# srihari-humbarwadi/retinanet-tensorflow2.x

Hardware: AMD Instinct MI355X
Metric: images/sec train, ResNet50-640 RetinaNet data-parallel step (encode + fwd + loss + bwd + clip + all-reduce + SGD/EMA); inference images/s under `infer` (higher is better)
Workload: dtype bf16; 1 GPU; ResNet50-640x640 bf16 training, 32 images/GPU (BASELINE configs[2] shard: global batch 32), resnet_initial frozen, single GPU; global_batch=32, parallelism=dp1, rccl_ranks=1, comm=torch, syncbn_messages=0

## Files before the change

retinanet-tensorflow2.x_amd/csrc/rn_train.hip:

```cpp
#include "rn_common.h"

#define TR_THREADS 256

struct bf8 { float v[8]; };
__device__ __forceinline__ bf8 unpack8(uint4 u) {
  bf8 r;
  r.v[0] = rn_bf16_to_f32((uint16_t)(u.x & 0xffffu)); r.v[1] = rn_bf16_to_f32((uint16_t)(u.x >> 16));
  r.v[2] = rn_bf16_to_f32((uint16_t)(u.y & 0xffffu)); r.v[3] = rn_bf16_to_f32((uint16_t)(u.y >> 16));
  r.v[4] = rn_bf16_to_f32((uint16_t)(u.z & 0xffffu)); r.v[5] = rn_bf16_to_f32((uint16_t)(u.z >> 16));
  r.v[6] = rn_bf16_to_f32((uint16_t)(u.w & 0xffffu)); r.v[7] = rn_bf16_to_f32((uint16_t)(u.w >> 16));
  return r;
}
__device__ __forceinline__ uint4 pack8(const bf8& r) {
  uint4 u;
  u.x = rn_pack_bf16x2(r.v[0], r.v[1]); u.y = rn_pack_bf16x2(r.v[2], r.v[3]);
  u.z = rn_pack_bf16x2(r.v[4], r.v[5]); u.w = rn_pack_bf16x2(r.v[6], r.v[7]);
  return u;
}
__device__ __forceinline__ float act_mask(float z, int act) {
  if (act == RN_ACT_RELU) return z > 0.0f ? 1.0f : 0.0f;
  if (act == RN_ACT_RELU6) return (z > 0.0f && z < 6.0f) ? 1.0f : 0.0f;
  return 1.0f;
}
__device__ __forceinline__ float act_mask_u(float u, int act) {
  if (act == RN_ACT_RELU) return u > 0.0f ? 1.0f : 0.0f;
  if (act == RN_ACT_RELU6) {
    const float ub = rn_rb(u);
    return (ub > 0.0f && ub < 6.0f) ? 1.0f : 0.0f;
  }
  return 1.0f;
}
__device__ __forceinline__ float act_deriv(float z, float u, int act) {
  if (act == RN_ACT_SWISH) {
    const float sg = 1.0f / (1.0f + __expf(-u));
    return sg + u * sg * (1.0f - sg);
  }
  return act_mask(z, act);
}

enum { G_GENERIC = 0, G_NONE = 1, G_U_RELU = 2, G_U_RELU6 = 3, G_Z_RELU = 4, G_Z_RELU6 = 5, G_SWISH = 6, G_MASK = 7,
       G_SWISH_RES = 8 };
__device__ __forceinline__ float bn_swish_input(float u, float res) { return rn_rb(rn_rb(u) + res); }
template <int G>
__device__ __forceinline__ float grad_gate(float dz, float z, float u, int act, bool from_u) {
  if (G == G_NONE || G == G_MASK) return dz;
  if (G == G_U_RELU) return u > 0.0f ? dz : 0.0f;
  if (G == G_U_RELU6) {
    const float ub = rn_rb(u);
    return (ub > 0.0f && ub < 6.0f) ? dz : 0.0f;
  }
  if (G == G_Z_RELU) return z > 0.0f ? dz : 0.0f;
  if (G == G_Z_RELU6) return (z > 0.0f && z < 6.0f) ? dz : 0.0f;
  if (G == G_SWISH || G == G_SWISH_RES) {
    const float sg = __builtin_amdgcn_rcpf(1.0f + __expf(-u));
    return dz * (sg + u * sg * (1.0f - sg));
  }
  return act == RN_ACT_NONE ? dz : dz * (from_u ? act_mask_u(u, act) : act_deriv(z, u, act));
}
static int bn_gate_mode(const rn_bn_problem* p) {
  if (p->act == RN_ACT_NONE) return G_NONE;
  int with_res = 0;
  for (int i = 0; i < p->num_segments; ++i) with_res += p->seg[i].residual ? 1 : 0;
  if (with_res != 0 && with_res != p->num_segments) return G_GENERIC;
  if (p->act == RN_ACT_SWISH) return with_res ? G_SWISH_RES : G_SWISH;
  if (with_res == 0) return p->act == RN_ACT_RELU ? G_U_RELU : (p->act == RN_ACT_RELU6 ? G_U_RELU6 : G_GENERIC);
  int with_mask = 0;
  for (int i = 0; i < p->num_segments; ++i) with_mask += p->seg[i].act_mask ? 1 : 0;
  if (with_mask == p->num_segments && (p->act == RN_ACT_RELU || p->act == RN_ACT_RELU6)) return G_MASK;
  return p->act == RN_ACT_RELU ? G_Z_RELU : (p->act == RN_ACT_RELU6 ? G_Z_RELU6 : G_GENERIC);
}
#define BN_DISPATCH_GATE(mode_, CALL_)                  \
  switch (mode_) {                                      \
    case G_NONE: CALL_(G_NONE); break;                  \
    case G_U_RELU: CALL_(G_U_RELU); break;              \
    case G_U_RELU6: CALL_(G_U_RELU6); break;            \
    case G_Z_RELU: CALL_(G_Z_RELU); break;              \
    case G_Z_RELU6: CALL_(G_Z_RELU6); break;            \
    case G_SWISH: CALL_(G_SWISH); break;                \
    case G_MASK: CALL_(G_MASK); break;                  \
    case G_SWISH_RES: CALL_(G_SWISH_RES); break;        \
    default: CALL_(G_GENERIC); break;                   \
  }

static int tr_blocks(long long items, int cap = 8192) {
  long long b = rn_cdiv(items, TR_THREADS);
  if (b > cap) b = cap;
  if (b < 1) b = 1;
  return (int)b;
}

struct BnSegDev {
  const uint4* y; uint4* z; const uint4* residual; const uint4* dz; uint4* dy; uint4* dres;
  float* sums; float* fwd; float* bsums;
  const float* gamma; const float* beta; float* moving_mean; float* moving_var; float* dgamma; float* dbeta;
  long long P;
  int C, dres_accumulate, chunks, rows_per_chunk;
  int slab_groups, nslab;
  const float* sample_scale; long long rows_per_sample;
  unsigned char* mask;
  float* colsum;
};
struct BnArgs {
  int nseg, act, bessel, mode, fuse_finalize;
  int chunk_u;
  float eps, momentum, count_scale;
  float* ws;
  long long ws_off[RN_CONV_MAX_SEGMENTS];
  int ks[RN_CONV_MAX_SEGMENTS];
  long long cnt_off[RN_CONV_MAX_SEGMENTS], slot_off[RN_CONV_MAX_SEGMENTS], total_bytes;
  BnSegDev seg[RN_CONV_MAX_SEGMENTS];
};
#define BN_KS_MAX 32
#define BN_KS_CHUNKS 512

template <int G, int SGT = 0>
__global__ void __launch_bounds__(TR_THREADS) bn_colreduce_kernel(const BnArgs a) {
  const BnSegDev& s = a.seg[blockIdx.z];
  const int chunk = blockIdx.x;
  const int slab = blockIdx.y;
  if (chunk >= s.chunks || slab >= s.nslab) return;
  const int C8 = s.C >> 3;
  const int SG = SGT ? SGT : s.slab_groups, RL = TR_THREADS / SG;
  const int rl = threadIdx.x / SG, cg = threadIdx.x - rl * SG;
  const int c8 = slab * SG + cg;
  const bool live = c8 < C8 && rl < RL;
  const long long r0 = (long long)chunk * s.rows_per_chunk;
  long long r1 = r0 + s.rows_per_chunk;
  if (r1 > s.P) r1 = s.P;
  float s0[8], s1[8];
#pragma unroll
  for (int q = 0; q < 8; ++q) s0[q] = s1[q] = 0.0f;
  float mean[8], istd[8], scq[8], shq[8];
  if (G >= 0 && live) {
#pragma unroll
    for (int q = 0; q < 8; ++q) {
      mean[q] = s.fwd[0 * s.C + c8 * 8 + q];
      istd[q] = s.fwd[1 * s.C + c8 * 8 + q];
      scq[q] = s.fwd[2 * s.C + c8 * 8 + q];
      shq[q] = s.fwd[3 * s.C + c8 * 8 + q];
    }
  }
  if (live) {
    for (long long r = r0 + rl; r < r1; r += RL) {
      const long long o = r * C8 + c8;
      const bf8 y = unpack8(s.y[o]);
      if (G < 0) {
#pragma unroll
        for (int q = 0; q < 8; ++q) {
          s0[q] += y.v[q];
          s1[q] += y.v[q] * y.v[q];
        }
      } else {
        const bf8 dz = unpack8(s.dz[o]);
        const bool from_u = !s.residual && (a.act == RN_ACT_RELU || a.act == RN_ACT_RELU6);
        constexpr bool need_z = G == G_Z_RELU || G == G_Z_RELU6 || G == G_GENERIC;
        bf8 z;
        if (need_z && (G != G_GENERIC || (a.act != RN_ACT_NONE && a.act != RN_ACT_SWISH && !from_u))) z = unpack8(s.z[o]);
        unsigned bits = 0xffu;
        if (G == G_MASK) bits = s.mask[o];
        const bool swish_res = G == G_SWISH_RES || (G == G_GENERIC && a.act == RN_ACT_SWISH && s.residual != nullptr);
        bf8 res;
        if (swish_res) res = unpack8(s.residual[o]);
        float m = 1.0f;
        if (s.sample_scale) m = s.sample_scale[(int)r / (int)s.rows_per_sample];
#pragma unroll
        for (int q = 0; q < 8; ++q) {
          float u = y.v[q] * scq[q] + shq[q];
          if (swish_res) u = bn_swish_input(u, res.v[q]);
          float g = grad_gate<G < 0 ? 0 : G>(dz.v[q], z.v[q], u, a.act, from_u) * m;
          if (G == G_MASK) g = ((bits >> q) & 1u) ? g : 0.0f;
          s0[q] += g;
          s1[q] += g * ((y.v[q] - mean[q]) * istd[q]);
        }
      }
    }
  }
  __shared__ float red[SGT == 8 ? 2 * 32 * 65 : 2 * (TR_THREADS * 8 + TR_THREADS)];
  const int W = SG * 8 + 1;
  if (rl < RL) {
#pragma unroll
    for (int q = 0; q < 8; ++q) {
      red[rl * W + cg * 8 + q] = s0[q];
      red[RL * W + rl * W + cg * 8 + q] = s1[q];
    }
  }
  __syncthreads();
  for (int t = threadIdx.x; t < 2 * SG * 8; t += TR_THREADS) {
    const int which = t >= SG * 8 ? 1 : 0, c = t - which * SG * 8;
    float v = 0.0f;
    for (int r = 0; r < RL; ++r) v += red[which * RL * W + r * W + c];
    const int ch = slab * SG * 8 + c;
    if (ch < s.C) a.ws[a.ws_off[blockIdx.z] + ((long long)chunk * 2 + which) * s.C + ch] = v;
  }
}

static void bn_slab_plan(int C8, int chunks, int* slab_groups, int* nslab) {
  const int old_n = (C8 + 7) / 8;
  auto score = [&](int n) {
    const int g = (C8 + n - 1) / n;
    return (double)C8 * (TR_THREADS / g) / ((double)n * TR_THREADS);
  };
  *slab_groups = C8 < 8 ? C8 : 8;
  *nslab = old_n;
  if (C8 >= 8 && (double)C8 / (8.0 * old_n) >= 0.95) return;
  double best = 0.0;
  for (int n = 1; n <= old_n; ++n) {
    const int g = (C8 + n - 1) / n;
    if (g > 64 || (g < 8 && n > 1)) continue;
    if (score(n) > best) best = score(n);
  }
  for (int n = 1; n <= old_n; ++n) {
    const int g = (C8 + n - 1) / n;
    if (g > 64 || (g < 8 && n > 1) || score(n) < best - 0.01) continue;
    if ((long long)chunks * n >= 512 || C8 < 8) {
      *slab_groups = g;
      *nslab = n;
      return;
    }
  }
}

__device__ __forceinline__ void bn_finalize_channel(const BnArgs& a, const BnSegDev& s, int c, double sum, double sumsq) {
  const double n = (double)s.P * (double)a.count_scale;
  const double mean = sum / n;
  double var = sumsq / n - mean * mean;
  if (var < 0.0) var = 0.0;
  const float istd = (float)(1.0 / sqrt(var + (double)a.eps));
  const float sc = s.gamma[c] * istd;
  s.fwd[0 * s.C + c] = (float)mean;
  s.fwd[1 * s.C + c] = istd;
  s.fwd[2 * s.C + c] = sc;
  s.fwd[3 * s.C + c] = s.beta[c] - (float)mean * sc;
  if (s.moving_mean) {
    const double vm = a.bessel && n > 1.0 ? var * n / (n - 1.0) : var;
    s.moving_mean[c] = s.moving_mean[c] * a.momentum + (float)mean * (1.0f - a.momentum);
    s.moving_var[c] = s.moving_var[c] * a.momentum + (float)vm * (1.0f - a.momentum);
  }
}

template <int CH>
__global__ void __launch_bounds__(1024) bn_colreduce_final_kernel(const BnArgs a) {
  constexpr int LANES = 1024 / CH, PER = LANES / 16;
  const BnSegDev& s = a.seg[blockIdx.y];
  __shared__ double red[2][LANES][CH + 1];
  __shared__ double red2[2][16][CH + 1];
  const int cl = threadIdx.x & (CH - 1), lane = threadIdx.x / CH;
  const int c = blockIdx.x * CH + cl;
  double t0 = 0.0, t1 = 0.0;
  if (c < s.C) {
    const float* p = a.ws + a.ws_off[blockIdx.y];
#pragma unroll 8
    for (int k = lane; k < s.chunks; k += LANES) {
      t0 += (double)p[((long long)k * 2 + 0) * s.C + c];
      t1 += (double)p[((long long)k * 2 + 1) * s.C + c];
    }
  }
  red[0][lane][cl] = t0;
  red[1][lane][cl] = t1;
  __syncthreads();
  if (threadIdx.x < 2 * 16 * CH) {
    const int which = threadIdx.x / (16 * CH), rem = threadIdx.x - which * (16 * CH);
    const int grp = rem / CH, ch = rem - grp * CH;
    double t = 0.0;
#pragma unroll
    for (int j = 0; j < PER; ++j) t += red[which][grp * PER + j][ch];
    red2[which][grp][ch] = t;
  }
  __syncthreads();
  if (threadIdx.x < 2 * CH) {
    const int which = threadIdx.x / CH, ch = threadIdx.x - which * CH;
    const int cc = blockIdx.x * CH + ch;
    if (cc < s.C) {
      double t = 0.0;
#pragma unroll
      for (int j = 0; j < 16; ++j) t += red2[which][j][ch];
      float* out = a.mode == 0 ? s.sums : s.bsums;
      out[which * s.C + cc] = (float)t;
      if (a.mode == 1) {
        float* gp = which == 0 ? s.dbeta : s.dgamma;
        if (gp) gp[cc] = (float)t;
      }
      red2[which][0][ch] = (double)(float)t;
    }
  }
  if (a.fuse_finalize) {
    __syncthreads();
    if (threadIdx.x < CH && c < s.C) bn_finalize_channel(a, s, c, red2[0][0][cl], red2[1][0][cl]);
  }
}

typedef unsigned bn_u32x2_t __attribute__((ext_vector_type(2)));
__global__ void __launch_bounds__(1024) bn_colreduce_final_split_kernel(const BnArgs a) {
  const BnSegDev& s = a.seg[blockIdx.y];
  const int ks = a.ks[blockIdx.y], part = blockIdx.z;
  if (part >= ks || (int)blockIdx.x * 16 >= s.C) return;
  __shared__ double red[16][2][16];
  __shared__ unsigned s_old;
  const int col = threadIdx.x & 3, lane = threadIdx.x >> 2, wave = threadIdx.x >> 6;
  const int c = blockIdx.x * 16 + col * 4;
  double t[8];
#pragma unroll
  for (int q = 0; q < 8; ++q) t[q] = 0.0;
  if (c < s.C) {
    const float* p = a.ws + a.ws_off[blockIdx.y] + c;
    const int per = (s.chunks + ks - 1) / ks;
    const int k1 = (part + 1) * per < s.chunks ? (part + 1) * per : s.chunks;
#pragma unroll 2
    for (int k = part * per + lane; k < k1; k += 256) {
      const float4 v0 = *(const float4*)(p + ((long long)k * 2 + 0) * s.C);
      const float4 v1 = *(const float4*)(p + ((long long)k * 2 + 1) * s.C);
      t[0] += (double)v0.x; t[1] += (double)v0.y; t[2] += (double)v0.z; t[3] += (double)v0.w;
      t[4] += (double)v1.x; t[5] += (double)v1.y; t[6] += (double)v1.z; t[7] += (double)v1.w;
    }
  }
#pragma unroll
  for (int m = 4; m < 64; m <<= 1)
#pragma unroll
    for (int q = 0; q < 8; ++q) t[q] += __shfl_xor(t[q], m, 64);
  if ((threadIdx.x & 63) < 4) {
#pragma unroll
    for (int q = 0; q < 8; ++q) red[wave][q >> 2][col * 4 + (q & 3)] = t[q];
  }
  __syncthreads();
  const int which = (threadIdx.x >> 4) & 1, ch = threadIdx.x & 15;
  double r = 0.0;
  if (threadIdx.x < 32) {
#pragma unroll
    for (int j = 0; j < 16; ++j) r += red[j][which][ch];
  }
  if (ks > 1) {
    char* const slots = (char*)a.ws + a.slot_off[blockIdx.y] + (size_t)blockIdx.x * ks * 256;
    if (threadIdx.x < 64) {
      if (threadIdx.x < 32) {
        const __amdgpu_buffer_rsrc_t rs = __builtin_amdgcn_make_buffer_rsrc((void*)(slots + part * 256), 0, 256, 0x00020000);
        const unsigned long long bits = __builtin_bit_cast(unsigned long long, r);
        __builtin_amdgcn_raw_buffer_store_b64(bn_u32x2_t{(unsigned)bits, (unsigned)(bits >> 32)}, rs, threadIdx.x * 8, 0, 16);
      }
      asm volatile("s_waitcnt vmcnt(0)" ::: "memory");
      if (threadIdx.x == 0) {
        unsigned* const cnt = (unsigned*)((char*)a.ws + a.cnt_off[blockIdx.y]) + blockIdx.x;
        const unsigned old = __hip_atomic_fetch_add(cnt, 1u, __ATOMIC_RELAXED, __HIP_MEMORY_SCOPE_AGENT);
        if (old == (unsigned)(ks - 1)) __hip_atomic_store(cnt, 0u, __ATOMIC_RELAXED, __HIP_MEMORY_SCOPE_AGENT);
        s_old = old;
      }
    }
    __syncthreads();
    if (s_old != (unsigned)(ks - 1)) return;
    if (threadIdx.x < 32) {
      const __amdgpu_buffer_rsrc_t rs = __builtin_amdgcn_make_buffer_rsrc((void*)slots, 0, ks * 256, 0x00020000);
      bn_u32x2_t pv[BN_KS_MAX];
#pragma unroll
      for (int j = 0; j < BN_KS_MAX; ++j) pv[j] = __builtin_amdgcn_raw_buffer_load_b64(rs, j * 256 + threadIdx.x * 8, 0, 16);
      r = 0.0;
#pragma unroll
      for (int j = 0; j < BN_KS_MAX; ++j)
        r += __builtin_bit_cast(double, ((unsigned long long)pv[j].y << 32) | pv[j].x);
    }
  }
  if (threadIdx.x < 32) {
    const int cc = blockIdx.x * 16 + ch;
    if (cc < s.C) {
      float* out = a.mode == 0 ? s.sums : s.bsums;
      out[which * s.C + cc] = (float)r;
      if (a.mode == 1) {
        float* gp = which == 0 ? s.dbeta : s.dgamma;
        if (gp) gp[cc] = (float)r;
      }
    }
    red[0][which][ch] = (double)(float)r;
  }
  if (a.fuse_finalize) {
    __syncthreads();
    const int cc = blockIdx.x * 16 + threadIdx.x;
    if (threadIdx.x < 16 && cc < s.C) bn_finalize_channel(a, s, cc, red[0][0][threadIdx.x], red[0][1][threadIdx.x]);
  }
}

__global__ void bn_finalize_kernel(const BnArgs a) {
  const BnSegDev& s = a.seg[blockIdx.y];
  const int c = blockIdx.x * blockDim.x + threadIdx.x;
  if (c >= s.C) return;
  bn_finalize_channel(a, s, c, (double)s.sums[c], (double)s.sums[s.C + c]);
}

#define BN_ELEMENTWISE_RANGE() BN_ELEMENTWISE_RANGE_(false)
#define BN_ELEMENTWISE_RANGE_(keep_)                                                                  \
  long long first, last, step;                                                                        \
  if (a.chunk_u > 0) {                                                                                \
    const long long span = 256ll * a.chunk_u;                                                         \
    first = blockIdx.x * span + threadIdx.x;                                                          \
    last = (blockIdx.x + 1) * span < total ? (blockIdx.x + 1) * span : total;                         \
    step = 256;                                                                                       \
    if (first >= last) {                                                                              \
      if (!(keep_) || blockIdx.x * span >= total) return;    \
      first = last;                                                                                   \
    }                                                                                                 \
  } else {                                                                                            \
    const long long nthreads = (long long)gridDim.x * blockDim.x;                                     \
    step = nthreads / C8 * C8;                                                                        \
    first = blockIdx.x * (long long)blockDim.x + threadIdx.x;                                         \
    last = total;                                                                                     \
    if (first >= step) return;                                                                        \
  }

__global__ void __launch_bounds__(TR_THREADS) bn_apply_kernel(const BnArgs a) {
  const BnSegDev& s = a.seg[blockIdx.y];
  const int C8 = s.C >> 3;
  const long long total = s.P * C8;
  BN_ELEMENTWISE_RANGE();
  const int c8 = (int)(first % C8);
  float sc[8], sh[8];
#pragma unroll
  for (int q = 0; q < 8; ++q) {
    sc[q] = s.fwd[2 * s.C + c8 * 8 + q];
    sh[q] = s.fwd[3 * s.C + c8 * 8 + q];
  }
  for (long long i = first; i < last; i += step) {
    const bf8 y = unpack8(s.y[i]);
    bf8 o;
    bf8 res;
    if (s.residual) res = unpack8(s.residual[i]);
    const float m = s.sample_scale ? s.sample_scale[(int)(i / C8) / (int)s.rows_per_sample] : 1.0f;
    const bool swish = a.act == RN_ACT_SWISH;
#pragma unroll
    for (int q = 0; q < 8; ++q) o.v[q] = y.v[q] * sc[q] + sh[q];
    if (s.residual != nullptr || s.sample_scale != nullptr || swish) {
#pragma unroll
      for (int q = 0; q < 8; ++q) o.v[q] = rn_rb(o.v[q]);
    }
    if (s.sample_scale) {
#pragma unroll
      for (int q = 0; q < 8; ++q) o.v[q] = rn_rb(o.v[q] * m);
    }
    if (s.residual) {
#pragma unroll
      for (int q = 0; q < 8; ++q) o.v[q] += res.v[q];
      if (swish) {
#pragma unroll
        for (int q = 0; q < 8; ++q) o.v[q] = rn_rb(o.v[q]);
      }
    }
    rn_apply_act_n<8>(o.v, a.act);
    const uint4 zp = pack8(o);
    s.z[i] = zp;
    if (s.mask) {
      const bf8 zs = unpack8(zp);
      unsigned bits = 0u;
      if (a.act == RN_ACT_RELU) {
#pragma unroll
        for (int q = 0; q < 8; ++q) bits |= (zs.v[q] > 0.0f ? 1u : 0u) << q;
      } else if (a.act == RN_ACT_RELU6) {
#pragma unroll
        for (int q = 0; q < 8; ++q) bits |= ((zs.v[q] > 0.0f && zs.v[q] < 6.0f) ? 1u : 0u) << q;
      } else {
        bits = 0xffu;
      }
      s.mask[i] = (unsigned char)bits;
    }
  }
}

template <int G>
__global__ void __launch_bounds__(TR_THREADS) bn_bwd_apply_kernel(const BnArgs a) {
  const BnSegDev& s = a.seg[blockIdx.y];
  const int C8 = s.C >> 3;
  const long long total = s.P * C8;
  const float inv_n = (float)(1.0 / ((double)s.P * (double)a.count_scale));
  const bool colsum = s.colsum != nullptr;
  BN_ELEMENTWISE_RANGE_(colsum);
  const int c8 = a.chunk_u > 0 ? (int)(threadIdx.x % C8) : (int)(first % C8);
  float mean[8], istd[8], sc[8], shq[8], k1[8], k2[8];
#pragma unroll
  for (int q = 0; q < 8; ++q) {
    const int c = c8 * 8 + q;
    mean[q] = s.fwd[0 * s.C + c];
    istd[q] = s.fwd[1 * s.C + c];
    sc[q] = s.fwd[2 * s.C + c];
    shq[q] = s.fwd[3 * s.C + c];
    k1[q] = s.bsums[c] * inv_n;
    k2[q] = s.bsums[s.C + c] * inv_n;
  }
  float cs[8];
#pragma unroll
  for (int q = 0; q < 8; ++q) cs[q] = 0.0f;
  for (long long i = first; i < last; i += step) {
    const bf8 y = unpack8(s.y[i]);
    const bf8 dz = unpack8(s.dz[i]);
    const bool from_u = !s.residual && (a.act == RN_ACT_RELU || a.act == RN_ACT_RELU6);
    constexpr bool need_z = G == G_Z_RELU || G == G_Z_RELU6 || G == G_GENERIC;
    bf8 z;
    if (need_z && (G != G_GENERIC || (a.act != RN_ACT_NONE && a.act != RN_ACT_SWISH && !from_u))) z = unpack8(s.z[i]);
    const float m = s.sample_scale ? s.sample_scale[(int)(i / C8) / (int)s.rows_per_sample] : 1.0f;
    unsigned bits = 0xffu;
    if (G == G_MASK) bits = s.mask[i];
    const bool swish_res = G == G_SWISH_RES || (G == G_GENERIC && a.act == RN_ACT_SWISH && s.residual != nullptr);
    bf8 res;
    if (swish_res) res = unpack8(s.residual[i]);
    bf8 g, o;
#pragma unroll
    for (int q = 0; q < 8; ++q) {
      float u = y.v[q] * sc[q] + shq[q];
      if (swish_res) u = bn_swish_input(u, res.v[q]);
      g.v[q] = grad_gate<G>(dz.v[q], z.v[q], u, a.act, from_u);
      if (G == G_MASK) g.v[q] = ((bits >> q) & 1u) ? g.v[q] : 0.0f;
      const float xh = (y.v[q] - mean[q]) * istd[q];
      o.v[q] = sc[q] * (g.v[q] * m - k1[q] - xh * k2[q]);
    }
    const uint4 dyp = pack8(o);
    s.dy[i] = dyp;
    if (colsum) {
      const bf8 st = unpack8(dyp);
#pragma unroll
      for (int q = 0; q < 8; ++q) cs[q] += st.v[q];
    }
    if (s.dres) {
      if (s.dres_accumulate) {
        const bf8 old = unpack8(s.dres[i]);
#pragma unroll
        for (int q = 0; q < 8; ++q) g.v[q] += old.v[q];
      }
      s.dres[i] = pack8(g);
    }
  }
  if (colsum) {
    __shared__ float red[TR_THREADS][9];
#pragma unroll
    for (int q = 0; q < 8; ++q) red[threadIdx.x][q] = cs[q];
    __syncthreads();
    if ((int)threadIdx.x < C8) {
      float t[8];
#pragma unroll
      for (int q = 0; q < 8; ++q) t[q] = 0.0f;
      for (int j = threadIdx.x; j < TR_THREADS; j += C8)
#pragma unroll
        for (int q = 0; q < 8; ++q) t[q] += red[j][q];
      float* dst = s.colsum + ((long long)blockIdx.x * 2) * s.C + threadIdx.x * 8;
#pragma unroll
      for (int q = 0; q < 8; ++q) dst[q] = t[q];
    }
  }
}

static int bn_chunks_of(const rn_bn_segment& s, int mode, int* rows_per_chunk) {
  const long long want_chunks = 2048 / rn_cdiv(s.C, 64) < 256 ? 256 : 2048 / rn_cdiv(s.C, 64);
  long long rpc = rn_cdiv(rn_cdiv(s.P, want_chunks), 32) * 32;
  if (rpc < 32) rpc = 32;
  if (rows_per_chunk) *rows_per_chunk = (int)rpc;
  int chunks = (int)rn_cdiv(s.P, rpc);
  if (mode == 0 && s.ext_chunks > 0) chunks = s.ext_chunks;
  if (mode == 1 && s.ext_chunks_bwd > 0) chunks = s.ext_chunks_bwd;
  return chunks;
}

static int bn_fill(const rn_bn_problem* p, BnArgs& a, int need_ws, int mode = 1) {
  if (!p || p->num_segments < 1 || p->num_segments > RN_CONV_MAX_SEGMENTS) return -1;
  a.nseg = p->num_segments; a.act = p->act; a.bessel = p->bessel; a.mode = 0; a.fuse_finalize = 0; a.chunk_u = 0;
  a.eps = p->eps; a.momentum = p->momentum; a.count_scale = p->count_scale > 0 ? p->count_scale : 1.0f;
  long long off = 0;
  for (int i = 0; i < p->num_segments; ++i) {
    const rn_bn_segment& s = p->seg[i];
    if (s.P <= 0 || s.C <= 0 || (s.C % 8)) return -1;
    BnSegDev& d = a.seg[i];
    d.y = (const uint4*)s.y; d.z = (uint4*)s.z; d.residual = (const uint4*)s.residual;
    d.dz = (const uint4*)s.dz; d.dy = (uint4*)s.dy; d.dres = (uint4*)s.dres;
    d.sums = s.sums; d.fwd = s.fwd; d.bsums = s.bsums; d.gamma = s.gamma; d.beta = s.beta;
    d.moving_mean = s.moving_mean; d.moving_var = s.moving_var; d.dgamma = s.dgamma; d.dbeta = s.dbeta;
    d.P = s.P; d.C = s.C; d.dres_accumulate = s.dres_accumulate;
    d.sample_scale = s.sample_scale; d.rows_per_sample = s.rows_per_sample > 0 ? s.rows_per_sample : 1;
    d.mask = (unsigned char*)s.act_mask;
    d.colsum = s.dy_colsum_partial;
    if (s.sample_scale && p->act == RN_ACT_SWISH) return -1;
    d.chunks = bn_chunks_of(s, mode, &d.rows_per_chunk);
    bn_slab_plan(s.C / 8, d.chunks, &d.slab_groups, &d.nslab);
    a.ws_off[i] = off;
    off += (long long)d.chunks * 2 * s.C;
  }
  long long other = 0;
  for (int i = 0; i < p->num_segments; ++i) other += (long long)bn_chunks_of(p->seg[i], 1 - mode, nullptr) * 2 * p->seg[i].C;
  long long tail = ((off > other ? off : other) * 4 + 255) / 256 * 256;
  for (int i = 0; i < p->num_segments; ++i) {
    a.cnt_off[i] = tail;
    tail += rn_cdiv(p->seg[i].C, 16) * 4;
  }
  tail = (tail + 255) / 256 * 256;
  for (int i = 0; i < p->num_segments; ++i) {
    const int ch = a.seg[i].chunks;
    int ks = ch > BN_KS_CHUNKS ? (int)rn_cdiv(ch, 256) : 1;
    if (ks > BN_KS_MAX) ks = BN_KS_MAX;
    a.ks[i] = ks;
    a.slot_off[i] = tail;
    if (ks > 1) tail += rn_cdiv(p->seg[i].C, 16) * ks * 256;
  }
  a.total_bytes = tail;
  (void)need_ws;
  return 0;
}

extern "C" size_t rn_bn_workspace_bytes(const rn_bn_problem* p) {
  size_t need = 0;
  for (int mode = 0; mode < 2; ++mode) {
    BnArgs a;
    if (bn_fill(p, a, 1, mode)) return 0;
    if ((size_t)a.total_bytes > need) need = (size_t)a.total_bytes;
  }
  return need;
}

extern "C" int rn_bn_workspace_init(const rn_bn_problem* p, void* ws, size_t ws_bytes, void* stream) {
  BnArgs a;
  RN_CHECK_ARG(p && bn_fill(p, a, 1, 0) == 0, "rn_bn_workspace_init: bad problem (C %% 8 == 0, 1..10 segments)");
  const size_t need = rn_bn_workspace_bytes(p);
  if (!ws || ws_bytes < need) {
    rn_set_error("rn_bn_workspace_init: workspace too small (%zu < %zu)", ws_bytes, need);
    return RN_ENOMEM;
  }
  const long long begin = a.cnt_off[0];
  long long end = begin;
  for (int i = 0; i < p->num_segments; ++i) end = a.cnt_off[i] + rn_cdiv(p->seg[i].C, 16) * 4;
  RN_CHECK_HIP(hipMemsetAsync((char*)ws + begin, 0, (size_t)(end - begin), (hipStream_t)stream));
  return RN_OK;
}

extern "C" size_t rn_bn_partial_offset_bytes(const rn_bn_problem* p, int segment) {
  BnArgs a;
  if (bn_fill(p, a, 1, 0) || segment < 0 || segment >= a.nseg) return 0;
  return (size_t)a.ws_off[segment] * sizeof(float);
}

extern "C" size_t rn_bn_bwd_partial_offset_bytes(const rn_bn_problem* p, int segment) {
  BnArgs a;
  if (bn_fill(p, a, 1, 1) || segment < 0 || segment >= a.nseg) return 0;
  return (size_t)a.ws_off[segment] * sizeof(float);
}

static int bn_colreduce(const rn_bn_problem* p, int mode, void* ws, size_t ws_bytes, hipStream_t st,
                        const char* fn, int fuse_finalize = 0) {
  BnArgs a;
  RN_CHECK_ARG(bn_fill(p, a, 1, mode) == 0, "%s: bad problem (C %% 8 == 0, 1..10 segments)", fn);
  int n_ext = 0;
  for (int i = 0; i < p->num_segments; ++i)
    n_ext += ((mode == 0 && p->seg[i].ext_chunks > 0) || (mode == 1 && p->seg[i].ext_chunks_bwd > 0)) ? 1 : 0;
  RN_CHECK_ARG(n_ext == 0 || n_ext == p->num_segments, "%s: ext_chunks must be set on all segments or none", fn);
  if (mode == 1 && n_ext) {
    RN_CHECK_ARG(bn_gate_mode(p) == G_U_RELU, "%s: ext_chunks_bwd needs act = relu without residual inputs", fn);
    for (int i = 0; i < p->num_segments; ++i)
      RN_CHECK_ARG(!p->seg[i].sample_scale, "%s: ext_chunks_bwd with sample_scale", fn);
  }
  if (!ws || ws_bytes < rn_bn_workspace_bytes(p)) {
    rn_set_error("%s: workspace too small", fn);
    return RN_ENOMEM;
  }
  a.mode = mode;
  a.fuse_finalize = fuse_finalize;
  if (fuse_finalize)
    for (int i = 0; i < a.nseg; ++i)
      RN_CHECK_ARG(a.seg[i].fwd && a.seg[i].gamma && a.seg[i].beta, "%s: null tensor", fn);
  a.ws = (float*)ws;
  int max_chunks = 0, max_slabs = 0, max_c = 0;
  for (int i = 0; i < a.nseg; ++i) {
    const BnSegDev& s = a.seg[i];
    RN_CHECK_ARG(s.y && (mode == 0 ? s.sums != nullptr : (s.dz && s.bsums && s.fwd)), "%s: null tensor", fn);
    RN_CHECK_ARG(mode == 0 || a.act == RN_ACT_NONE || s.z || s.mask, "%s: z needed for the activation mask", fn);
    RN_CHECK_ARG(mode == 0 || bn_gate_mode(p) != G_GENERIC || a.act == RN_ACT_SWISH || !s.residual || s.z,
                 "%s: z needed for the activation mask", fn);
    if (s.chunks > max_chunks) max_chunks = s.chunks;
    if (s.nslab > max_slabs) max_slabs = s.nslab;
    if (s.C > max_c) max_c = s.C;
  }
  if (n_ext == 0) {
    const dim3 grid(max_chunks, max_slabs, a.nseg), block(TR_THREADS);
    bool all8 = true;
    for (int i = 0; i < a.nseg; ++i) all8 = all8 && a.seg[i].slab_groups == 8;
    if (mode == 0) {
      if (all8) hipLaunchKernelGGL((bn_colreduce_kernel<-1, 8>), grid, block, 0, st, a);
      else hipLaunchKernelGGL((bn_colreduce_kernel<-1, 0>), grid, block, 0, st, a);
    } else {
#define BN_CALL_(G_)                                                                       \
  if (all8) hipLaunchKernelGGL((bn_colreduce_kernel<G_, 8>), grid, block, 0, st, a);       \
  else hipLaunchKernelGGL((bn_colreduce_kernel<G_, 0>), grid, block, 0, st, a)
      BN_DISPATCH_GATE(bn_gate_mode(p), BN_CALL_)
#undef BN_CALL_
    }
    RN_CHECK_LAUNCH();
  }
  int max_ks = 1;
  for (int i = 0; i < a.nseg; ++i) max_ks = a.ks[i] > max_ks ? a.ks[i] : max_ks;
  if (max_ks > 1 && (((uintptr_t)a.ws) & 15) == 0)
    hipLaunchKernelGGL(bn_colreduce_final_split_kernel, dim3((max_c + 15) / 16, a.nseg, max_ks), dim3(1024), 0, st, a);
  else
    hipLaunchKernelGGL(bn_colreduce_final_kernel<16>, dim3((max_c + 15) / 16, a.nseg), dim3(1024), 0, st, a);
  RN_CHECK_LAUNCH();
  return RN_OK;
}

extern "C" int rn_bn_stats(const rn_bn_problem* p, void* ws, size_t ws_bytes, void* stream) {
  return bn_colreduce(p, 0, ws, ws_bytes, (hipStream_t)stream, "rn_bn_stats");
}
extern "C" int rn_bn_stats_finalize(const rn_bn_problem* p, void* ws, size_t ws_bytes, void* stream) {
  return bn_colreduce(p, 0, ws, ws_bytes, (hipStream_t)stream, "rn_bn_stats_finalize", 1);
}
extern "C" int rn_bn_bwd_reduce(const rn_bn_problem* p, void* ws, size_t ws_bytes, void* stream) {
  return bn_colreduce(p, 1, ws, ws_bytes, (hipStream_t)stream, "rn_bn_bwd_reduce");
}

extern "C" int rn_bn_finalize(const rn_bn_problem* p, void* stream) {
  BnArgs a;
  RN_CHECK_ARG(bn_fill(p, a, 0) == 0, "rn_bn_finalize: bad problem");
  int max_c = 0;
  for (int i = 0; i < a.nseg; ++i) {
    RN_CHECK_ARG(a.seg[i].sums && a.seg[i].fwd && a.seg[i].gamma && a.seg[i].beta, "rn_bn_finalize: null tensor");
    if (a.seg[i].C > max_c) max_c = a.seg[i].C;
  }
  hipLaunchKernelGGL(bn_finalize_kernel, dim3((max_c + 255) / 256, a.nseg), dim3(256), 0, (hipStream_t)stream, a);
  RN_CHECK_LAUNCH();
  return RN_OK;
}

#ifndef RN_BN_CHUNK_U
#define RN_BN_CHUNK_U 8
#endif
static int bn_elementwise_grid(BnArgs& a, long long max_units) {
  static_assert(TR_THREADS == 256, "BN_ELEMENTWISE_RANGE assumes 256 threads");
  bool chunk = RN_BN_CHUNK_U > 0;
  for (int i = 0; i < a.nseg; ++i) chunk = chunk && 256 % (a.seg[i].C >> 3) == 0;
  const long long blocks = rn_cdiv(max_units, 256ll * (RN_BN_CHUNK_U > 0 ? RN_BN_CHUNK_U : 1));
  if (chunk && blocks < (1ll << 31)) {
    a.chunk_u = RN_BN_CHUNK_U;
    return (int)blocks;
  }
  a.chunk_u = 0;
  return tr_blocks(max_units, 4096);
}

extern "C" int rn_bn_apply(const rn_bn_problem* p, void* stream) {
  BnArgs a;
  RN_CHECK_ARG(bn_fill(p, a, 0) == 0, "rn_bn_apply: bad problem");
  long long mx = 0;
  for (int i = 0; i < a.nseg; ++i) {
    RN_CHECK_ARG(a.seg[i].y && a.seg[i].z && a.seg[i].fwd, "rn_bn_apply: null tensor");
    const long long t = a.seg[i].P * (a.seg[i].C / 8);
    if (t > mx) mx = t;
  }
  hipLaunchKernelGGL(bn_apply_kernel, dim3(bn_elementwise_grid(a, mx), a.nseg), dim3(TR_THREADS), 0, (hipStream_t)stream, a);
  RN_CHECK_LAUNCH();
  return RN_OK;
}

extern "C" int rn_bn_bwd_colsum_chunks(const rn_bn_problem* p, int segment) {
  BnArgs a;
  if (bn_fill(p, a, 0) || segment < 0 || segment >= a.nseg) return 0;
  long long mx = 0;
  for (int i = 0; i < a.nseg; ++i) {
    const long long t = a.seg[i].P * (a.seg[i].C / 8);
    if (t > mx) mx = t;
  }
  bn_elementwise_grid(a, mx);
  if (a.chunk_u <= 0) return 0;
  return (int)rn_cdiv(a.seg[segment].P * (a.seg[segment].C / 8), 256ll * a.chunk_u);
}

extern "C" int rn_bn_bwd_apply(const rn_bn_problem* p, void* stream) {
  BnArgs a;
  RN_CHECK_ARG(bn_fill(p, a, 0) == 0, "rn_bn_bwd_apply: bad problem");
  long long mx = 0;
  for (int i = 0; i < a.nseg; ++i) {
    RN_CHECK_ARG(a.seg[i].y && a.seg[i].dz && a.seg[i].dy && a.seg[i].fwd && a.seg[i].bsums,
                 "rn_bn_bwd_apply: null tensor");
    RN_CHECK_ARG(a.act == RN_ACT_NONE || a.seg[i].z || a.seg[i].mask, "rn_bn_bwd_apply: z needed for the activation mask");
    RN_CHECK_ARG(bn_gate_mode(p) != G_GENERIC || a.act == RN_ACT_SWISH || !a.seg[i].residual || a.seg[i].z,
                 "rn_bn_bwd_apply: z needed for the activation mask");
    const long long t = a.seg[i].P * (a.seg[i].C / 8);
    if (t > mx) mx = t;
  }
  {
    const dim3 grid(bn_elementwise_grid(a, mx), a.nseg), block(TR_THREADS);
    for (int i = 0; i < a.nseg; ++i)
      RN_CHECK_ARG(!a.seg[i].colsum || a.chunk_u > 0,
                   "rn_bn_bwd_apply: dy_colsum_partial needs the chunked form (rn_bn_bwd_colsum_chunks() > 0)");
#define BN_CALL_(G_) hipLaunchKernelGGL(bn_bwd_apply_kernel<G_>, grid, block, 0, (hipStream_t)stream, a)
    BN_DISPATCH_GATE(bn_gate_mode(p), BN_CALL_)
#undef BN_CALL_
  }
  RN_CHECK_LAUNCH();
  return RN_OK;
}

__global__ void __launch_bounds__(TR_THREADS)
act_bwd_kernel(const uint4* __restrict__ dz, const uint4* __restrict__ z, uint4* __restrict__ dy, long long n8,
               int act) {
  for (long long i = blockIdx.x * (long long)blockDim.x + threadIdx.x; i < n8;
       i += (long long)gridDim.x * blockDim.x) {
    bf8 g = unpack8(dz[i]);
    const bf8 zz = unpack8(z[i]);
#pragma unroll
    for (int q = 0; q < 8; ++q) g.v[q] *= act_mask(zz.v[q], act);
    dy[i] = pack8(g);
  }
}

__global__ void __launch_bounds__(TR_THREADS)
cast_f32_bf16_kernel(const float4* __restrict__ x, uint2* __restrict__ y, long long n4) {
  for (long long i = blockIdx.x * (long long)blockDim.x + threadIdx.x; i < n4;
       i += (long long)gridDim.x * blockDim.x) {
    const float4 v = x[i];
    uint2 o;
    o.x = rn_pack_bf16x2(v.x, v.y);
    o.y = rn_pack_bf16x2(v.z, v.w);
    y[i] = o;
  }
}
__global__ void __launch_bounds__(TR_THREADS)
cast_pad_kernel(const float* __restrict__ x, uint2* __restrict__ y, long long P, int C, int Cpad) {
  const int q = Cpad / 4;
  const long long total = P * q;
  for (long long i = blockIdx.x * (long long)blockDim.x + threadIdx.x; i < total;
       i += (long long)gridDim.x * blockDim.x) {
    const long long r = i / q;
    const int c = (int)(i - r * q) * 4;
    float v[4];
#pragma unroll
    for (int u = 0; u < 4; ++u) v[u] = (c + u) < C ? x[r * C + c + u] : 0.0f;
    uint2 o;
    o.x = rn_pack_bf16x2(v[0], v[1]);
    o.y = rn_pack_bf16x2(v[2], v[3]);
    y[i] = o;
  }
}
extern "C" int rn_cast_pad_f32_to_bf16(const float* x, void* y, int64_t P, int C, int Cpad, void* stream) {
  RN_CHECK_ARG(x && y && P > 0 && C > 0 && Cpad >= C && Cpad % 4 == 0, "rn_cast_pad_f32_to_bf16: bad argument");
  hipLaunchKernelGGL(cast_pad_kernel, dim3(tr_blocks(P * (Cpad / 4))), dim3(TR_THREADS), 0, (hipStream_t)stream, x,
                     (uint2*)y, (long long)P, C, Cpad);
  RN_CHECK_LAUNCH();
  return RN_OK;
}
extern "C" int rn_cast_f32_to_bf16(const float* x, void* y, int64_t n, void* stream) {
  RN_CHECK_ARG(x && y && n > 0 && n % 4 == 0, "rn_cast_f32_to_bf16: bad argument (n %% 4 == 0)");
  hipLaunchKernelGGL(cast_f32_bf16_kernel, dim3(tr_blocks(n / 4)), dim3(TR_THREADS), 0, (hipStream_t)stream,
                     (const float4*)x, (uint2*)y, (long long)(n / 4));
  RN_CHECK_LAUNCH();
  return RN_OK;
}

__global__ void __launch_bounds__(TR_THREADS)
reduce_rows_kernel(const float* __restrict__ src, int rows, long long row_stride, int n, float add, float* __restrict__ dst) {
  const int c = blockIdx.x * blockDim.x + threadIdx.x;
  if (c >= n) return;
  float s = 0.0f;
  for (int r = 0; r < rows; ++r) s += src[r * row_stride + c];
  dst[c] = s + add;
}
extern "C" int rn_reduce_rows_f32(const float* src, int rows, int64_t row_stride, int n, float add, float* dst, void* stream) {
  RN_CHECK_ARG(src && dst && rows > 0 && n > 0 && row_stride >= 0, "rn_reduce_rows_f32: bad argument");
  hipLaunchKernelGGL(reduce_rows_kernel, dim3((n + TR_THREADS - 1) / TR_THREADS), dim3(TR_THREADS), 0, (hipStream_t)stream,
                     src, rows, (long long)row_stride, n, add, dst);
  RN_CHECK_LAUNCH();
  return RN_OK;
}

__global__ void __launch_bounds__(TR_THREADS)
upsample_zero_kernel(const uint4* __restrict__ x, uint4* __restrict__ y, int N, int H, int W, int C8, int Ho,
                     int Wo) {
  const long long total = (long long)N * Ho * Wo * C8;
  for (long long i = blockIdx.x * (long long)blockDim.x + threadIdx.x; i < total;
       i += (long long)gridDim.x * blockDim.x) {
    const RnIdx4 d_ = rn_decode4(i, C8, Wo, Ho, rn_decode_mode(total, C8));
    const int c = d_.c, ox = d_.x, oy = d_.y, n = d_.n;
    uint4 v = make_uint4(0u, 0u, 0u, 0u);
    if (!(ox & 1) && !(oy & 1) && (oy >> 1) < H && (ox >> 1) < W)
      v = x[(((long long)n * H + (oy >> 1)) * W + (ox >> 1)) * C8 + c];
    y[i] = v;
  }
}
extern "C" int rn_upsample_zero2x(const void* x, void* y, int N, int H, int W, int C, int Ho, int Wo,
                                  void* stream) {
  RN_CHECK_ARG(x && y && N > 0 && H > 0 && W > 0 && C % 8 == 0 && Ho >= 2 * H - 1 && Wo >= 2 * W - 1,
               "rn_upsample_zero2x: bad argument");
  hipLaunchKernelGGL(upsample_zero_kernel, dim3(tr_blocks((long long)N * Ho * Wo * (C / 8))), dim3(TR_THREADS), 0,
                     (hipStream_t)stream, (const uint4*)x, (uint4*)y, N, H, W, C / 8, Ho, Wo);
  RN_CHECK_LAUNCH();
  return RN_OK;
}

__global__ void __launch_bounds__(TR_THREADS)
scatter_add2x_kernel(const uint4* __restrict__ x, uint4* __restrict__ y, int N, int H, int W, int C8, int Ho, int Wo) {
  const long long total = (long long)N * H * W * C8;
  for (long long i = blockIdx.x * (long long)blockDim.x + threadIdx.x; i < total;
       i += (long long)gridDim.x * blockDim.x) {
    const RnIdx4 d_ = rn_decode4(i, C8, W, H, rn_decode_mode(total, C8));
    const int c = d_.c, w = d_.x, h = d_.y, n = d_.n;
    if (2 * h >= Ho || 2 * w >= Wo) continue;
    const long long o = (((long long)n * Ho + 2 * h) * Wo + 2 * w) * C8 + c;
    const bf8 a = unpack8(x[i]), b = unpack8(y[o]);
    bf8 r;
#pragma unroll
    for (int q = 0; q < 8; ++q) r.v[q] = a.v[q] + b.v[q];
    y[o] = pack8(r);
  }
}
extern "C" int rn_scatter_add2x(const void* x, void* y, int N, int H, int W, int C, int Ho, int Wo, int accumulate,
                                void* stream) {
  RN_CHECK_ARG(x && y && N > 0 && H > 0 && W > 0 && C % 8 == 0 && Ho >= 2 * H - 1 && Wo >= 2 * W - 1,
               "rn_scatter_add2x: bad argument");
  if (!accumulate) return rn_upsample_zero2x(x, y, N, H, W, C, Ho, Wo, stream);
  hipLaunchKernelGGL(scatter_add2x_kernel, dim3(tr_blocks((long long)N * H * W * (C / 8))), dim3(TR_THREADS), 0,
                     (hipStream_t)stream, (const uint4*)x, (uint4*)y, N, H, W, C / 8, Ho, Wo);
  RN_CHECK_LAUNCH();
  return RN_OK;
}

__global__ void __launch_bounds__(TR_THREADS)
depth_to_space2x_kernel(const uint4* __restrict__ x, uint4* __restrict__ y, int N, int H, int W, int C8, int accumulate) {
  const long long total = (long long)N * H * W * 4 * C8;
  for (long long i = blockIdx.x * (long long)blockDim.x + threadIdx.x; i < total;
       i += (long long)gridDim.x * blockDim.x) {
    const RnIdx4 d_ = rn_decode4(i, C8, 4 * W, H, rn_decode_mode(total, C8));
    const int c = d_.c, ph = d_.x & 3, w = d_.x >> 2, h = d_.y, n = d_.n;
    const long long o = (((long long)n * 2 * H + 2 * h + (ph >> 1)) * 2 * W + 2 * w + (ph & 1)) * C8 + c;
    uint4 v = x[i];
    if (accumulate) {
      const bf8 a = unpack8(v), b = unpack8(y[o]);
      bf8 r;
#pragma unroll
      for (int q = 0; q < 8; ++q) r.v[q] = a.v[q] + b.v[q];
      v = pack8(r);
    }
    y[o] = v;
  }
}
extern "C" int rn_depth_to_space2x(const void* x, void* y, int N, int H, int W, int C, int accumulate, void* stream) {
  RN_CHECK_ARG(x && y && N > 0 && H > 0 && W > 0 && C > 0 && C % 8 == 0, "rn_depth_to_space2x: bad argument");
  hipLaunchKernelGGL(depth_to_space2x_kernel, dim3(tr_blocks((long long)N * H * W * 4 * (C / 8))), dim3(TR_THREADS), 0,
                     (hipStream_t)stream, (const uint4*)x, (uint4*)y, N, H, W, C / 8, accumulate);
  RN_CHECK_LAUNCH();
  return RN_OK;
}

extern "C" int rn_act_bwd(const void* dz, const void* z, void* dy, int64_t n, int act, void* stream) {
  RN_CHECK_ARG(dz && z && dy && n > 0 && n % 8 == 0, "rn_act_bwd: bad argument");
  RN_CHECK_ARG(act != RN_ACT_SWISH, "rn_act_bwd: swish' needs the pre-activation, which is not an argument (only z is)");
  hipLaunchKernelGGL(act_bwd_kernel, dim3(tr_blocks(n / 8)), dim3(TR_THREADS), 0, (hipStream_t)stream,
                     (const uint4*)dz, (const uint4*)z, (uint4*)dy, (long long)(n / 8), act);
  RN_CHECK_LAUNCH();
  return RN_OK;
}

__global__ void __launch_bounds__(TR_THREADS)
maxpool_bwd_kernel(const uint4* __restrict__ x, const uint4* __restrict__ dy, uint4* __restrict__ dx, int N, int H,
                   int W, int C8, int k, int stride, int pt, int pl, int Ho, int Wo, int accumulate) {
  const long long total = (long long)N * H * W * C8;
  for (long long i = blockIdx.x * (long long)blockDim.x + threadIdx.x; i < total;
       i += (long long)gridDim.x * blockDim.x) {
    const RnIdx4 d_ = rn_decode4(i, C8, W, H, rn_decode_mode(total, C8));
    const int c = d_.c, ix = d_.x, iy = d_.y, n = d_.n;
    const bf8 me = unpack8(x[i]);
    bf8 g;
    if (accumulate) g = unpack8(dx[i]);
    else {
#pragma unroll
      for (int q = 0; q < 8; ++q) g.v[q] = 0.0f;
    }
    int oy0 = (iy + pt - (k - 1) + stride - 1) / stride;
    if (iy + pt - (k - 1) < 0) oy0 = 0;
    int ox0 = (ix + pl - (k - 1) + stride - 1) / stride;
    if (ix + pl - (k - 1) < 0) ox0 = 0;
    const int oy1 = (iy + pt) / stride, ox1 = (ix + pl) / stride;
    for (int oy = oy0; oy <= oy1 && oy < Ho; ++oy)
      for (int ox = ox0; ox <= ox1 && ox < Wo; ++ox) {
        const int my_r = iy - (oy * stride - pt), my_s = ix - (ox * stride - pl);
        bool win[8];
#pragma unroll
        for (int q = 0; q < 8; ++q) win[q] = true;
        for (int r = 0; r < k; ++r) {
          const int yy = oy * stride - pt + r;
          if ((unsigned)yy >= (unsigned)H) continue;
          for (int s = 0; s < k; ++s) {
            const int xx = ox * stride - pl + s;
            if ((unsigned)xx >= (unsigned)W || (r == my_r && s == my_s)) continue;
            const bf8 v = unpack8(x[(((long long)n * H + yy) * W + xx) * C8 + c]);
            const bool before = r < my_r || (r == my_r && s < my_s);
#pragma unroll
            for (int q = 0; q < 8; ++q)
              if (before ? (v.v[q] >= me.v[q]) : (v.v[q] > me.v[q])) win[q] = false;
          }
        }
        const bf8 d = unpack8(dy[(((long long)n * Ho + oy) * Wo + ox) * C8 + c]);
#pragma unroll
        for (int q = 0; q < 8; ++q)
          if (win[q]) g.v[q] += d.v[q];
      }
    dx[i] = pack8(g);
  }
// ... 268 lines not shown
```

Measured before the change: 1123 images/s.

## Flatten BN split-reduce grid and shrink blocks to 256 threads with batched loads

Reworks the BN column-reduce final split kernel to use a flattened 1D grid indexed by per-segment item offsets, so blocks that would exit early because a segment has fewer channels or splits are never launched. Blocks drop from 1024 to 256 threads; each thread issues four rows of loads up front and then covers the remaining stride-256 rows, accumulating into the same 16-slot shared reduction. The last-arriving block's cross-split merge now loads the partial slots with 64 threads in two halves. This is meant to cut wasted block launches and improve latency hiding, at the cost of more per-thread serial work and a segment-lookup loop in each block.

```diff
diff --git a/retinanet-tensorflow2.x_amd/csrc/rn_train.hip b/retinanet-tensorflow2.x_amd/csrc/rn_train.hip
--- a/retinanet-tensorflow2.x_amd/csrc/rn_train.hip
+++ b/retinanet-tensorflow2.x_amd/csrc/rn_train.hip
@@ -107,6 +107,7 @@
   float* ws;
   long long ws_off[RN_CONV_MAX_SEGMENTS];
   int ks[RN_CONV_MAX_SEGMENTS];
+  int item0[RN_CONV_MAX_SEGMENTS + 1];
   long long cnt_off[RN_CONV_MAX_SEGMENTS], slot_off[RN_CONV_MAX_SEGMENTS], total_bytes;
   BnSegDev seg[RN_CONV_MAX_SEGMENTS];
 };
@@ -290,36 +291,50 @@
 }
 
 typedef unsigned bn_u32x2_t __attribute__((ext_vector_type(2)));
-__global__ void __launch_bounds__(1024) bn_colreduce_final_split_kernel(const BnArgs a) {
-  const BnSegDev& s = a.seg[blockIdx.y];
-  const int ks = a.ks[blockIdx.y], part = blockIdx.z;
-  if (part >= ks || (int)blockIdx.x * 16 >= s.C) return;
+__global__ void __launch_bounds__(256) bn_colreduce_final_split_kernel(const BnArgs a) {
+  int sg = 0;
+  while (sg + 1 < a.nseg && (int)blockIdx.x >= a.item0[sg + 1]) ++sg;
+  const BnSegDev& s = a.seg[sg];
+  const int ks = a.ks[sg], nblk = (s.C + 15) >> 4;
+  const int item = (int)blockIdx.x - a.item0[sg], part = item / nblk, blk = item - part * nblk;
   __shared__ double red[16][2][16];
   __shared__ unsigned s_old;
   const int col = threadIdx.x & 3, lane = threadIdx.x >> 2, wave = threadIdx.x >> 6;
-  const int c = blockIdx.x * 16 + col * 4;
-  double t[8];
-#pragma unroll
-  for (int q = 0; q < 8; ++q) t[q] = 0.0;
-  if (c < s.C) {
-    const float* p = a.ws + a.ws_off[blockIdx.y] + c;
-    const int per = (s.chunks + ks - 1) / ks;
-    const int k1 = (part + 1) * per < s.chunks ? (part + 1) * per : s.chunks;
-#pragma unroll 2
-    for (int k = part * per + lane; k < k1; k += 256) {
-      const float4 v0 = *(const float4*)(p + ((long long)k * 2 + 0) * s.C);
-      const float4 v1 = *(const float4*)(p + ((long long)k * 2 + 1) * s.C);
-      t[0] += (double)v0.x; t[1] += (double)v0.y; t[2] += (double)v0.z; t[3] += (double)v0.w;
-      t[4] += (double)v1.x; t[5] += (double)v1.y; t[6] += (double)v1.z; t[7] += (double)v1.w;
-    }
-  }
-#pragma unroll
-  for (int m = 4; m < 64; m <<= 1)
-#pragma unroll
-    for (int q = 0; q < 8; ++q) t[q] += __shfl_xor(t[q], m, 64);
-  if ((threadIdx.x & 63) < 4) {
-#pragma unroll
-    for (int q = 0; q < 8; ++q) red[wave][q >> 2][col * 4 + (q & 3)] = t[q];
+  const int c = blk * 16 + col * 4;
+  const float* p = a.ws + a.ws_off[sg] + (c < s.C ? c : 0);
+  const int per = (s.chunks + ks - 1) / ks;
+  const int k0 = part * per + lane;
+  const int k1 = c >= s.C ? 0 : ((part + 1) * per < s.chunks ? (part + 1) * per : s.chunks);
+  float4 v[4][2];
+#pragma unroll
+  for (int j = 0; j < 4; ++j) {
+    const int k = k0 + 64 * j < k1 ? k0 + 64 * j : 0;
+#pragma unroll
+    for (int h = 0; h < 2; ++h) v[j][h] = *(const float4*)(p + ((long long)k * 2 + h) * s.C);
+  }
+  __builtin_amdgcn_sched_barrier(0);
+#pragma unroll
+  for (int j = 0; j < 4; ++j) {
+    const bool row = k0 + 64 * j < k1;
+#pragma unroll
+    for (int h = 0; h < 2; ++h) {
+      double t[4];
+      t[0] = 0.0 + (double)(row ? v[j][h].x : 0.0f); t[1] = 0.0 + (double)(row ? v[j][h].y : 0.0f);
+      t[2] = 0.0 + (double)(row ? v[j][h].z : 0.0f); t[3] = 0.0 + (double)(row ? v[j][h].w : 0.0f);
+      for (int k = k0 + 64 * j + 256; k < k1; k += 256) {
+        const float4 w = *(const float4*)(p + ((long long)k * 2 + h) * s.C);
+        t[0] += (double)w.x; t[1] += (double)w.y; t[2] += (double)w.z; t[3] += (double)w.w;
+      }
+#pragma unroll
+      for (int m = 4; m < 64; m <<= 1)
+#pragma unroll
+        for (int q = 0; q < 4; ++q) t[q] += __shfl_xor(t[q], m, 64);
+      if ((threadIdx.x & 63) < 4) {
+#pragma unroll
+        for (int q = 0; q < 4; ++q) red[4 * j + wave][h][col * 4 + q] = t[q];
+      }
+      __builtin_amdgcn_sched_barrier(0);
+    }
   }
   __syncthreads();
   const int which = (threadIdx.x >> 4) & 1, ch = threadIdx.x & 15;
@@ -329,7 +344,7 @@
     for (int j = 0; j < 16; ++j) r += red[j][which][ch];
   }
   if (ks > 1) {
-    char* const slots = (char*)a.ws + a.slot_off[blockIdx.y] + (size_t)blockIdx.x * ks * 256;
+    char* const slots = (char*)a.ws + a.slot_off[sg] + (size_t)blk * ks * 256;
     if (threadIdx.x < 64) {
       if (threadIdx.x < 32) {
         const __amdgpu_buffer_rsrc_t rs = __builtin_amdgcn_make_buffer_rsrc((void*)(slots + part * 256), 0, 256, 0x00020000);
@@ -338,7 +353,7 @@
       }
       asm volatile("s_waitcnt vmcnt(0)" ::: "memory");
       if (threadIdx.x == 0) {
-        unsigned* const cnt = (unsigned*)((char*)a.ws + a.cnt_off[blockIdx.y]) + blockIdx.x;
+        unsigned* const cnt = (unsigned*)((char*)a.ws + a.cnt_off[sg]) + blk;
         const unsigned old = __hip_atomic_fetch_add(cnt, 1u, __ATOMIC_RELAXED, __HIP_MEMORY_SCOPE_AGENT);
         if (old == (unsigned)(ks - 1)) __hip_atomic_store(cnt, 0u, __ATOMIC_RELAXED, __HIP_MEMORY_SCOPE_AGENT);
         s_old = old;
@@ -346,19 +361,31 @@
     }
     __syncthreads();
     if (s_old != (unsigned)(ks - 1)) return;
+    bn_u32x2_t pv[BN_KS_MAX / 2];
+    if (threadIdx.x < 64) {
+      const __amdgpu_buffer_rsrc_t rs = __builtin_amdgcn_make_buffer_rsrc((void*)slots, 0, ks * 256, 0x00020000);
+      const int half = threadIdx.x >> 5;
+#pragma unroll
+      for (int j = 0; j < BN_KS_MAX / 2; ++j)
+        pv[j] = __builtin_amdgcn_raw_buffer_load_b64(rs, (half * (BN_KS_MAX / 2) + j) * 256 + (threadIdx.x & 31) * 8, 0, 16);
+      if (half) {
+#pragma unroll
+        for (int j = 0; j < BN_KS_MAX / 2; ++j)
+          red[j][which][ch] = __builtin_bit_cast(double, ((unsigned long long)pv[j].y << 32) | pv[j].x);
+      }
+    }
+    __syncthreads();
     if (threadIdx.x < 32) {
-      const __amdgpu_buffer_rsrc_t rs = __builtin_amdgcn_make_buffer_rsrc((void*)slots, 0, ks * 256, 0x00020000);
-      bn_u32x2_t pv[BN_KS_MAX];
-#pragma unroll
-      for (int j = 0; j < BN_KS_MAX; ++j) pv[j] = __builtin_amdgcn_raw_buffer_load_b64(rs, j * 256 + threadIdx.x * 8, 0, 16);
       r = 0.0;
 #pragma unroll
-      for (int j = 0; j < BN_KS_MAX; ++j)
+      for (int j = 0; j < BN_KS_MAX / 2; ++j)
         r += __builtin_bit_cast(double, ((unsigned long long)pv[j].y << 32) | pv[j].x);
+#pragma unroll
+      for (int j = 0; j < BN_KS_MAX / 2; ++j) r += red[j][which][ch];
     }
   }
   if (threadIdx.x < 32) {
-    const int cc = blockIdx.x * 16 + ch;
+    const int cc = blk * 16 + ch;
     if (cc < s.C) {
       float* out = a.mode == 0 ? s.sums : s.bsums;
       out[which * s.C + cc] = (float)r;
@@ -371,7 +398,7 @@
   }
   if (a.fuse_finalize) {
     __syncthreads();
-    const int cc = blockIdx.x * 16 + threadIdx.x;
+    const int cc = blk * 16 + threadIdx.x;
     if (threadIdx.x < 16 && cc < s.C) bn_finalize_channel(a, s, cc, red[0][0][threadIdx.x], red[0][1][threadIdx.x]);
   }
 }
@@ -591,6 +618,8 @@
     a.slot_off[i] = tail;
     if (ks > 1) tail += rn_cdiv(p->seg[i].C, 16) * ks * 256;
   }
+  a.item0[0] = 0;
+  for (int i = 0; i < p->num_segments; ++i) a.item0[i + 1] = a.item0[i] + a.ks[i] * (int)rn_cdiv(p->seg[i].C, 16);
   a.total_bytes = tail;
   (void)need_ws;
   return 0;
@@ -686,7 +715,7 @@
   int max_ks = 1;
   for (int i = 0; i < a.nseg; ++i) max_ks = a.ks[i] > max_ks ? a.ks[i] : max_ks;
   if (max_ks > 1 && (((uintptr_t)a.ws) & 15) == 0)
-    hipLaunchKernelGGL(bn_colreduce_final_split_kernel, dim3((max_c + 15) / 16, a.nseg, max_ks), dim3(1024), 0, st, a);
+    hipLaunchKernelGGL(bn_colreduce_final_split_kernel, dim3(a.item0[a.nseg]), dim3(256), 0, st, a);
   else
     hipLaunchKernelGGL(bn_colreduce_final_kernel<16>, dim3((max_c + 15) / 16, a.nseg), dim3(1024), 0, st, a);
   RN_CHECK_LAUNCH();
```

After: 1120 images/s. No clear change (-0.2%).
